# bioinformatics-ua/polus

Hardware: AMD Instinct MI355X
Metric: train samples/sec BioBERT-base NER seq256 (higher is better)
Workload: dtype bf16; 1 GPU; BERT-base (L=12,H=768,A=12,I=3072,V=28996) token classification C=4, seq_len=256, 64 samples/GPU, AdamW lr 5e-5 wd 0.01 warm-up 10%, dropout 0.1 (hidden + attention) (BASELINE.json configs[2] per-GPU shape), random-init weights; global_batch=64, seq_len=256, parallelism=dp1, grad_allreduce=none

## Files before the change

### polus_amd/csrc/attention.hip

```cpp
#include "common.h"

namespace {

constexpr int D = 64;
constexpr int BLK = 64;
constexpr float MASK_NEG = -10000.0f;
constexpr float LOG2E = 1.4426950408889634f, LN2 = 0.6931471805599453f;

template <typename T> struct TileCfg;
template <> struct TileCfg<bf16_t> { static constexpr int RS = 160, EPC = 8, LOG_CPR = 3, NLOAD = 2; };
template <> struct TileCfg<float> { static constexpr int RS = 288, EPC = 4, LOG_CPR = 4, NLOAD = 4; };

template <typename T, int NT = 256>
__device__ __forceinline__ void tile_load(unsigned char* tile, const T* __restrict__ base, long ld, int row0,
                                          int nrows, int col0, int tid) {
    constexpr int LOG = TileCfg<T>::LOG_CPR;
#pragma unroll
    for (int k = 0; k < TileCfg<T>::NLOAD; ++k) {
        int c = tid + NT * k;
        int r = c >> LOG, ch = c & ((1 << LOG) - 1);
        uint4 v = make_uint4(0, 0, 0, 0);
        if (row0 + r < nrows)
            v = *reinterpret_cast<const uint4*>(base + (long)(row0 + r) * ld + col0 + ch * TileCfg<T>::EPC);
        *reinterpret_cast<uint4*>(tile + r * TileCfg<T>::RS + ch * 16) = v;
// ... 37 lines not shown

__device__ __forceinline__ void frag_from_acc(Frag<bf16_t>& f, const f32x4& t0, const f32x4& t1) {
    f.v[0] = (bf16_t)t0[0]; f.v[1] = (bf16_t)t0[1]; f.v[2] = (bf16_t)t0[2]; f.v[3] = (bf16_t)t0[3];
    f.v[4] = (bf16_t)t1[0]; f.v[5] = (bf16_t)t1[1]; f.v[6] = (bf16_t)t1[2]; f.v[7] = (bf16_t)t1[3];
}
__device__ __forceinline__ void frag_from_acc(Frag<float>& f, const f32x4& t0, const f32x4& t1) {
    f.v[0] = t0[0]; f.v[1] = t0[1]; f.v[2] = t0[2]; f.v[3] = t0[3];
    f.v[4] = t1[0]; f.v[5] = t1[1]; f.v[6] = t1[2]; f.v[7] = t1[3];
}

__device__ __forceinline__ float col_max(float v) { v = fmaxf(v, __shfl_xor(v, 16, 64)); return fmaxf(v, __shfl_xor(v, 32, 64)); }
__device__ __forceinline__ float col_sum(float v) { v += __shfl_xor(v, 16, 64); return v + __shfl_xor(v, 32, 64); }

template <typename T>
__device__ __forceinline__ void store_acc_T(T* __restrict__ out, long ld, int row, int col0, const f32x4 (&o)[4],
                                            float mul, int g, bool valid) {
    if (!valid) return;
#pragma unroll
    for (int dt = 0; dt < 4; ++dt) {
        float v[4] = {o[dt][0] * mul, o[dt][1] * mul, o[dt][2] * mul, o[dt][3] * mul};
        store4<T>(out + (long)row * ld + col0 + dt * 16 + 4 * g, v);
    }
}

struct AttnArgs {
    const void* qkv; const int32_t* mask; void* ctx; float* lse;
    const void* dctx; const float* delta; void* dqkv;
    int B, S, A, H;
    float scale;
    unsigned drop_thresh, drop_seed;
    float drop_inv;
    const PolusDyn* dyn;
    int debug;
};

__device__ __forceinline__ float key_bias(const int32_t* mask, int b, int S, int key) {
    if (key >= S) return -INFINITY;
    if (!mask) return 0.0f;
    return (1.0f - (float)mask[(long)b * S + key]) * MASK_NEG;
}

template <typename T, int NW>
__global__ __launch_bounds__(64 * NW) void attn_fwd_kernel(AttnArgs p) {
    if (p.drop_thresh) p.drop_seed = polus_eff_seed(p.drop_seed, p.dyn);
    constexpr int QB = 16 * NW, NT = 64 * NW;
    extern __shared__ __attribute__((aligned(16))) unsigned char smem[];
    unsigned char* Kc = smem;
    unsigned char* Vc = smem + QB * TileCfg<T>::RS;
    float* kbc = reinterpret_cast<float*>(smem + 2 * QB * TileCfg<T>::RS);
    const int tid = threadIdx.x, lane = tid & 63, wid = tid >> 6, i = lane & 15, g = lane >> 4;
    const int q0 = blockIdx.x * QB, h = blockIdx.y, b = blockIdx.z;
    const int S = p.S, H = p.H;
    const long ld = 3L * H;
    const T* qkv = static_cast<const T*>(p.qkv) + (long)b * S * ld;
    const int q = q0 + wid * 16 + i;
    const bool qvalid = q < S;

    Frag<T> qf[2];
#pragma unroll
    for (int sub = 0; sub < 2; ++sub)
        frag_global<T>(qf[sub], qkv + (long)q * ld + h * D + sub * 32 + 8 * g, qvalid);

    const float scale2 = p.scale * LOG2E;
    float m = -1e30f, l = 0.f;
    f32x4 o[4];
#pragma unroll
    for (int dt = 0; dt < 4; ++dt) o[dt] = (f32x4){0.f, 0.f, 0.f, 0.f};
// ... 117 lines not shown

    auto issue_block = [&](int j) {
        unsigned char* st = ring + (j & 3) * FWD_STAGE;
#pragma unroll
        for (int e = 0; e < PPW; ++e) {
            const int piece = wid + e * NW;
            const int row = min(j * BLK + (piece & 7) * 8 + r8, S - 1);
            dma16(qkv + (long)row * ld + (piece < 8 ? H : 2 * H) + h * D + src_chunk, st + piece * 1024);
        }
    };
    const int nblk = (S + BLK - 1) / BLK;
    if (p.mask)
        for (int k0 = wid * 64; k0 < S; k0 += 64 * NW)
            dma4(p.mask + (long)b * S + min(k0 + lane, S - 1), reinterpret_cast<unsigned char*>(kbc) + k0 * 4);
    {
        unsigned char* qs = ring + 3 * FWD_STAGE;
#pragma unroll
        for (int e = 0; e < 2; ++e) {
            const int piece = wid + e * NW;
            dma16(qkv + (long)min(q0 + piece * 8 + r8, S - 1) * ld + h * D + src_chunk, qs + piece * 1024);
        }
    }
#pragma unroll
    for (int j = 0; j < 3; ++j) if (j < nblk) issue_block(j);
    wait_blocks_left<PPW>(min(nblk, 3));
    __builtin_amdgcn_s_barrier();
    Frag<T> qf[2];
    {
        const int row = wid * 16 + i;
#pragma unroll
        for (int sub = 0; sub < 2; ++sub)
            qf[sub].v = *reinterpret_cast<const bf16x8*>(ring + 3 * FWD_STAGE + row * 128 + (((sub * 4 + g) ^ (row & 7)) * 16));
    }
    for (int t = tid; t < nblk * BLK; t += NT) {
        float bias = 0.0f;
        if (p.mask) bias = (1.0f - (float)reinterpret_cast<const int*>(kbc)[t]) * MASK_NEG;
        kbc[t] = t < S ? bias * LOG2E : -INFINITY;
    }
    wait_lgkm();
    __builtin_amdgcn_s_barrier();
    if (nblk > 3) issue_block(3);
    int issued = min(nblk, 4);

    const float scale2 = p.scale * LOG2E;
    float m = -1e30f, l = 0.f;
    f32x4 o[4];
#pragma unroll
    for (int dt = 0; dt < 4; ++dt) o[dt] = (f32x4){0.f, 0.f, 0.f, 0.f};
    const int kx = i & 7;
    const int k_off0 = i * 128 + ((g ^ kx) * 16), k_off1 = i * 128 + (((4 + g) ^ kx) * 16);
    const int vrow = 4 * g + (i >> 2), vx = vrow & 7;
    const int v_base = vrow * 128 + (i & 1) * 8, v_c = (i & 3) >> 1;

    for (int j0 = 0; j0 < nblk; j0 += 2) {
        const bool two = j0 + 1 < nblk;
        f32x4 s[2][4];
#pragma unroll
        for (int jj = 0; jj < 2; ++jj) {
            if (jj == 0 || two) {
                wait_blocks_left<PPW>(issued - 1 - (j0 + jj));
                __builtin_amdgcn_s_barrier();
                const unsigned char* Kt = ring + ((j0 + jj) & 3) * FWD_STAGE;
#pragma unroll
                for (int kt = 0; kt < 4; ++kt) {
                    s[jj][kt] = (f32x4){0.f, 0.f, 0.f, 0.f};
                    Frag<T> a0, a1;
                    a0.v = *reinterpret_cast<const bf16x8*>(Kt + kt * 2048 + k_off0);
                    a1.v = *reinterpret_cast<const bf16x8*>(Kt + kt * 2048 + k_off1);
                    mma16(s[jj][kt], a0, qf[0]);
                    mma16(s[jj][kt], a1, qf[1]);
                }
            } else {
#pragma unroll
                for (int kt = 0; kt < 4; ++kt) s[jj][kt] = (f32x4){-INFINITY, -INFINITY, -INFINITY, -INFINITY};
            }
        }
        float mx = -INFINITY;
#pragma unroll
        for (int jj = 0; jj < 2; ++jj)
            if (jj == 0 || two) {
#pragma unroll
                for (int kt = 0; kt < 4; ++kt) {
                    const f32x4 kb = *reinterpret_cast<const f32x4*>(kbc + (j0 + jj) * BLK + kt * 16 + 4 * g);
#pragma unroll
                    for (int r = 0; r < 4; ++r) s[jj][kt][r] = fmaf(s[jj][kt][r], scale2, kb[r]);
                    mx = fmaxf(mx, fmaxf(fmaxf(s[jj][kt][0], s[jj][kt][1]), fmaxf(s[jj][kt][2], s[jj][kt][3])));
                }
            }
        mx = col_max2(mx);
        const float m_new = fmaxf(m, mx);
        const float alpha = __builtin_amdgcn_exp2f(m - m_new);
        m = m_new;
        float rs = 0.f;
        Frag<T> pf[2][2];
#pragma unroll
        for (int jj = 0; jj < 2; ++jj) {
#pragma unroll
            for (int kt = 0; kt < 4; ++kt)
#pragma unroll
                for (int r = 0; r < 4; ++r) { s[jj][kt][r] = __builtin_amdgcn_exp2f(s[jj][kt][r] - m_new); rs += s[jj][kt][r]; }
            if (p.drop_thresh) {
                const unsigned rowb = (((unsigned)b * p.A + h) * S + (unsigned)q) * S + (j0 + jj) * BLK + 4 * g;
#pragma unroll
                for (int kt = 0; kt < 4; ++kt) {
                    float t4[4] = {s[jj][kt][0], s[jj][kt][1], s[jj][kt][2], s[jj][kt][3]};
                    polus_dropout_run<4>(t4, p.drop_seed, rowb + kt * 16, p.drop_thresh, p.drop_inv, (S & 3) == 0);
                    s[jj][kt] = (f32x4){t4[0], t4[1], t4[2], t4[3]};
                }
            }
            frag_from_acc(pf[jj][0], s[jj][0], s[jj][1]);
            frag_from_acc(pf[jj][1], s[jj][2], s[jj][3]);
        }
        l = l * alpha + rs;
#pragma unroll
        for (int dt = 0; dt < 4; ++dt)
#pragma unroll
            for (int r = 0; r < 4; ++r) o[dt][r] *= alpha;
#pragma unroll
        for (int jj = 0; jj < 2; ++jj) {
            if (jj == 0 || two) {
                const unsigned char* Vt = ring + ((j0 + jj) & 3) * FWD_STAGE + BLK * 128 + v_base;
#pragma unroll
                for (int ks = 0; ks < 2; ++ks)
#pragma unroll
                    for (int dt = 0; dt < 4; ++dt) {
                        const unsigned char* vp = Vt + ks * 4096 + (((2 * dt + v_c) ^ vx) * 16);
                        const s16x4 lo = lds_tr16(vp), hi = lds_tr16(vp + 16 * 128);
                        typedef short s16x8 __attribute__((ext_vector_type(8)));
                        const s16x8 w = {lo[0], lo[1], lo[2], lo[3], hi[0], hi[1], hi[2], hi[3]};
                        Frag<T> va;
                        va.v = __builtin_bit_cast(bf16x8, w);
                        mma16(o[dt], va, pf[jj][ks]);
                    }
            }
        }
        if (j0 + 4 < nblk) {
            wait_lgkm();
            __builtin_amdgcn_s_barrier();
            issue_block(j0 + 4);
            ++issued;
            if (j0 + 5 < nblk) { issue_block(j0 + 5); ++issued; }
        }
    }
    l = col_sum2(l);
    const float inv_l = 1.0f / l;
    wait_lgkm();
    __builtin_amdgcn_s_barrier();
    unsigned char* ot = ring + wid * 2048;
#pragma unroll
    for (int dt = 0; dt < 4; ++dt) {
        float v[4] = {o[dt][0] * inv_l, o[dt][1] * inv_l, o[dt][2] * inv_l, o[dt][3] * inv_l};
        store4<T>(reinterpret_cast<T*>(ot + i * 128 + (((2 * dt + (g >> 1)) ^ (i & 7)) * 16) + (g & 1) * 8), v);
    }
    wait_lgkm();
    T* ctx = static_cast<T*>(p.ctx) + (long)b * S * H;
#pragma unroll
    for (int t = 0; t < 2; ++t) {
        const int row = 8 * t + r8, qq = q0 + wid * 16 + row;
        const uint4 v = *reinterpret_cast<const uint4*>(ot + row * 128 + (lane & 7) * 16);
        if (qq < S) *reinterpret_cast<uint4*>(ctx + (long)qq * H + h * D + (((lane & 7) ^ (row & 7)) * 8)) = v;
    }
    if (q < S && g == 0) p.lse[((long)b * p.A + h) * S + q] = m * LN2 + __logf(l);
}

template <typename T, int NW>
__global__ __launch_bounds__(64 * NW) void attn_bwd_dq_kernel(AttnArgs p) {
    if (p.drop_thresh) p.drop_seed = polus_eff_seed(p.drop_seed, p.dyn);
    constexpr int QB = 16 * NW, NT = 64 * NW;
    extern __shared__ __attribute__((aligned(16))) unsigned char smem[];
    unsigned char* Kc = smem;
    unsigned char* Vc = smem + QB * TileCfg<T>::RS;
    float* kbc = reinterpret_cast<float*>(smem + 2 * QB * TileCfg<T>::RS);
    const int tid = threadIdx.x, lane = tid & 63, wid = tid >> 6, i = lane & 15, g = lane >> 4;
    const int q0 = blockIdx.x * QB, h = blockIdx.y, b = blockIdx.z;
    const int S = p.S, H = p.H;
    const long ld = 3L * H;
    const T* qkv = static_cast<const T*>(p.qkv) + (long)b * S * ld;
    const T* dctx = static_cast<const T*>(p.dctx) + (long)b * S * H;
// ... 192 lines not shown
template <int NW>
__global__ __launch_bounds__(64 * NW) void attn_bwd_fused_kernel(AttnArgs p) {
    typedef bf16_t T;
    constexpr int S = 16 * NW, NT = 64 * NW, RS = TileCfg<T>::RS, NKB = S / KBLK, TPW = 16 / NW;
    if (p.drop_thresh) p.drop_seed = polus_eff_seed(p.drop_seed, p.dyn);
    extern __shared__ __attribute__((aligned(16))) unsigned char smem[];
    unsigned char* Qc = smem;
    unsigned char* Oc = Qc + S * RS;
    unsigned char* Kc = Oc + S * RS;
    unsigned char* Vc = Kc + 2 * KBLK * RS;
    unsigned char* Ps = Vc + 2 * KBLK * RS;
    unsigned char* Ds = Ps + S * RSS;
    float* kbc = reinterpret_cast<float*>(Ds + S * RSS);
    const int tid = threadIdx.x, lane = tid & 63, wid = tid >> 6, i = lane & 15, g = lane >> 4;
    const int h = blockIdx.x, b = blockIdx.y;
    const int H = p.H;
    const long ld = 3L * H;
    const T* qkv = static_cast<const T*>(p.qkv) + (long)b * S * ld;
    const T* dctx = static_cast<const T*>(p.dctx) + (long)b * S * H;
    T* dqkv = static_cast<T*>(p.dqkv) + (long)b * S * ld;
    const int q = wid * 16 + i;

    auto load_kv = [&](int kb, int buf) {
        for (int c = tid; c < 2 * KBLK * 8; c += NT) {
            const int which = c >> 8, cc = c & 255, r = cc >> 3, ch = cc & 7;
            const uint4 v = *reinterpret_cast<const uint4*>(qkv + (long)(kb * KBLK + r) * ld + (1 + which) * H + h * D + ch * 8);
            *reinterpret_cast<uint4*>((which ? Vc : Kc) + (buf * KBLK + r) * RS + ch * 16) = v;
        }
    };
    tile_load<T, NT>(Qc, qkv, ld, 0, S, h * D, tid);
    tile_load<T, NT>(Oc, dctx, H, 0, S, h * D, tid);
    load_kv(0, 0);
    if (tid < S) kbc[tid] = key_bias(p.mask, b, S, tid) * LOG2E;

    Frag<T> qf[2], dof[2];
#pragma unroll
    for (int sub = 0; sub < 2; ++sub) {
        frag_global<T>(qf[sub], qkv + (long)q * ld + h * D + sub * 32 + 8 * g, true);
        frag_global<T>(dof[sub], dctx + (long)q * H + h * D + sub * 32 + 8 * g, true);
    }
    const long stat = ((long)b * p.A + h) * S + q;
    const float lse2 = p.lse[stat] * LOG2E;
    const float scale2 = p.scale * LOG2E;
    float dl = 0.f;
    {
        const T* ctx = static_cast<const T*>(p.ctx) + (long)b * S * H;
#pragma unroll
        for (int sub = 0; sub < 2; ++sub) {
            Frag<T> of;
            frag_global<T>(of, ctx + (long)q * H + h * D + sub * 32 + 8 * g, true);
#pragma unroll
            for (int j = 0; j < 8; ++j) dl += (float)of.v[j] * (float)dof[sub].v[j];
        }
        dl = col_sum(dl);
    }
    f32x4 dq[4];
#pragma unroll
    for (int dt = 0; dt < 4; ++dt) dq[dt] = (f32x4){0.f, 0.f, 0.f, 0.f};
    __syncthreads();

    for (int kb = 0; kb < NKB; ++kb) {
        const int cur = kb & 1;
        const unsigned char* Kt = Kc + cur * KBLK * RS;
        const unsigned char* Vt = Vc + cur * KBLK * RS;
        if (kb + 1 < NKB) load_kv(kb + 1, cur ^ 1);
        f32x4 s[2], dp[2];
#pragma unroll
        for (int kt = 0; kt < 2; ++kt) {
            s[kt] = (f32x4){0.f, 0.f, 0.f, 0.f};
            dp[kt] = (f32x4){0.f, 0.f, 0.f, 0.f};
#pragma unroll
            for (int sub = 0; sub < 2; ++sub) {
                Frag<T> a;
                frag_row<T>(a, Kt, kt * 16 + i, sub, g);
                mma16(s[kt], a, qf[sub]);
                frag_row<T>(a, Vt, kt * 16 + i, sub, g);
                mma16(dp[kt], a, dof[sub]);
            }
        }
        const unsigned rowb = (((unsigned)b * p.A + h) * S + (unsigned)q) * S + kb * KBLK + 4 * g;
#pragma unroll
        for (int kt = 0; kt < 2; ++kt) {
            float pd[4], dsv[4];
            bool keep[4] = {true, true, true, true};
            if (p.drop_thresh) {
                polus_keep4(p.drop_seed, rowb + kt * 16, p.drop_thresh, keep);
            }
#pragma unroll
            for (int r = 0; r < 4; ++r) {
                const float pr = __builtin_amdgcn_exp2f(fmaf(s[kt][r], scale2, kbc[kb * KBLK + kt * 16 + 4 * g + r]) - lse2);
                const float pk = keep[r] ? pr * p.drop_inv : 0.f;
                const float dpe = keep[r] ? dp[kt][r] * p.drop_inv : 0.f;
                pd[r] = pk;
                dsv[r] = pr * (dpe - dl) * p.scale;
                s[kt][r] = dsv[r];
            }
            const int st_off = kt * (S * 32) + q * 32 + ((g ^ ((q >> 2) & 3)) * 8);
            store4<T>(reinterpret_cast<T*>(Ps + st_off), pd);
// ... 5 lines not shown
#pragma unroll
            for (int dt = 0; dt < 4; ++dt) {
                Frag<T> ka;
                frag_tr(ka, Kt, 0, dt * 16, i, g);
                mma16(dq[dt], ka, dsb);
            }
        }
        __syncthreads();
#pragma unroll
        for (int e = 0; e < TPW; ++e) {
            const int t = wid * TPW + e;
            const int type = t >> 3, dt = (t >> 1) & 3, ktile = t & 1;
            const unsigned char* At = type ? Oc : Qc;
            const unsigned char* Bt = type ? Ps : Ds;
            f32x4 acc = (f32x4){0.f, 0.f, 0.f, 0.f};
#pragma unroll
            for (int qs = 0; qs < S / 32; ++qs) {
                Frag<T> a, bb;
                frag_tr(a, At, qs * 32, dt * 16, i, g);
                {
                    const unsigned char* bp = Bt + ktile * (S * 32) + (qs * 32 + 4 * g + (i >> 2)) * 32 + (((i & 3) ^ g) * 8);
                    const s16x4 lo = lds_tr16(bp), hi = lds_tr16(bp + 16 * 32);
                    typedef short s16x8 __attribute__((ext_vector_type(8)));
                    const s16x8 w = {lo[0], lo[1], lo[2], lo[3], hi[0], hi[1], hi[2], hi[3]};
                    bb.v = __builtin_bit_cast(bf16x8, w);
                }
                mma16(acc, a, bb);
            }
            float v[4] = {acc[0], acc[1], acc[2], acc[3]};
            store4<T>(dqkv + (long)(kb * KBLK + ktile * 16 + i) * ld + (type ? 2 * H : H) + h * D + dt * 16 + 4 * g, v);
        }
        __syncthreads();
    }
    store_acc_T<T>(dqkv, ld, q, h * D, dq, 1.0f, g, true);
}

typedef __attribute__((address_space(3))) unsigned char lds_u8;
typedef int v2i_t __attribute__((ext_vector_type(2)));
__device__ __forceinline__ unsigned lds_off(const unsigned char* p) { return (unsigned)(unsigned long)(const lds_u8*)p; }
template <int ROW16>
__device__ __forceinline__ void tr_pair_asm(Frag<bf16_t>& f, unsigned addr) {
    v2i_t lo, hi;
    asm volatile("ds_read_b64_tr_b16 %0, %2\n\tds_read_b64_tr_b16 %1, %2 offset:%3" : "=&v"(lo), "=&v"(hi) : "v"(addr), "n"(ROW16));
    typedef int v4i_t __attribute__((ext_vector_type(4)));
    const v4i_t w = {lo[0], lo[1], hi[0], hi[1]};
    f.v = __builtin_bit_cast(bf16x8, w);
}
__device__ __forceinline__ void ds_read128_asm(Frag<bf16_t>& f, unsigned addr) {
    typedef int v4i_t __attribute__((ext_vector_type(4)));
    v4i_t w;
    asm volatile("ds_read_b128 %0, %1" : "=&v"(w) : "v"(addr));
    f.v = __builtin_bit_cast(bf16x8, w);
}
__device__ __forceinline__ uint2 ds_read64_asm(unsigned addr) {
    v2i_t w;
    asm volatile("ds_read_b64 %0, %1" : "=&v"(w) : "v"(addr));
    return make_uint2((unsigned)w[0], (unsigned)w[1]);
}
__device__ __forceinline__ void lds_fence() {
    asm volatile("s_waitcnt lgkmcnt(0)" ::: "memory");
    __builtin_amdgcn_sched_barrier(0);
}
template <int R> __device__ __forceinline__ unsigned quad_bcast(unsigned v) {
    return (unsigned)__builtin_amdgcn_mov_dpp((int)v, R | (R << 2) | (R << 4) | (R << 6), 0xF, 0xF, true);
}


constexpr int Q64_KB = 64;
template <int NW> struct Q64Cfg {
    static constexpr int S = 16 * NW;
    static constexpr int OFF_O = S * 128, OFF_K = 2 * S * 128, OFF_V = OFF_K + Q64_KB * 128, OFF_P = OFF_V + Q64_KB * 128,
                         OFF_D = OFF_P + 4 * S * 32, OFF_B = OFF_D + 4 * S * 32, SMEM = OFF_B + S * 4;
};

template <int NW>
__global__ __launch_bounds__(64 * NW, 4) void attn_bwd_q64_kernel(AttnArgs p) {
    typedef bf16_t T;
    typedef Q64Cfg<NW> C;
    constexpr int S = C::S, NT = 64 * NW, NKB = S / Q64_KB;
    constexpr int KVP = 16 / NW;
    constexpr int COMBOS = NW >= 8 ? 1 : 8 / NW;
    constexpr int KTW = NW == 16 ? 2 : 4;
    if (p.drop_thresh) p.drop_seed = polus_eff_seed(p.drop_seed, p.dyn);
    extern __shared__ __attribute__((aligned(16))) unsigned char smem[];
    unsigned char* Qi = smem;
    unsigned char* Oi = smem + C::OFF_O;
    unsigned char* Kb = smem + C::OFF_K;
    unsigned char* Vb = smem + C::OFF_V;
    unsigned char* Ps = smem + C::OFF_P;
    unsigned char* Ds = smem + C::OFF_D;
    float* kbc = reinterpret_cast<float*>(smem + C::OFF_B);
    const int tid = threadIdx.x, lane = tid & 63, i = lane & 15, g = lane >> 4;
    const int wid = __builtin_amdgcn_readfirstlane(tid >> 6);
    const int h = blockIdx.x, b = blockIdx.y;
    const int H = p.H;
    const long ld = 3L * H;
    const T* qkv = static_cast<const T*>(p.qkv) + (long)b * S * ld;
    const T* dctx = static_cast<const T*>(p.dctx) + (long)b * S * H;
    T* dqkv = static_cast<T*>(p.dqkv) + (long)b * S * ld;
    const int q = wid * 16 + i;
    const int r8 = lane >> 3, src_chunk = ((lane & 7) ^ r8) * 8;

    auto issue_kv = [&](int kb) {
#pragma unroll
        for (int e = 0; e < KVP; ++e) {
            const int piece = wid + e * NW;
            const long row = (long)(kb * Q64_KB + (piece & 7) * 8 + r8) * ld + h * D + src_chunk;
            dma16(qkv + row + (piece < 8 ? H : 2 * H), (piece < 8 ? Kb : Vb) + (piece & 7) * 1024);
        }
    };
#pragma unroll
    for (int e = 0; e < 2; ++e) {
        const int piece = wid + e * NW;
        dma16(qkv + (long)(piece * 8 + r8) * ld + h * D + src_chunk, Qi + piece * 1024);
        dma16(dctx + (long)(piece * 8 + r8) * H + h * D + src_chunk, Oi + piece * 1024);
    }
    issue_kv(0);
    if (tid < S) kbc[tid] = key_bias(p.mask, b, S, tid) * LOG2E;
    const long stat = ((long)b * p.A + h) * S + q;
    const float lse2 = p.lse[stat] * LOG2E;
    const float scale2 = p.scale * LOG2E;
    Frag<T> of[2];
    {
        const T* ctx = static_cast<const T*>(p.ctx) + (long)b * S * H;
#pragma unroll
        for (int sub = 0; sub < 2; ++sub) frag_global<T>(of[sub], ctx + (long)q * H + h * D + sub * 32 + 8 * g, true);
    }
    wait_vm<0>();
    wait_lgkm();
    __builtin_amdgcn_s_barrier();
    const int qoff0 = q * 128 + ((g ^ (q & 7)) * 16), qoff1 = q * 128 + (((4 + g) ^ (q & 7)) * 16);
    float dl = 0.f;
    {
        Frag<T> dof[2];
        ds_read128_asm(dof[0], lds_off(Oi + qoff0));
        ds_read128_asm(dof[1], lds_off(Oi + qoff1));
        lds_fence();
#pragma unroll
        for (int sub = 0; sub < 2; ++sub)
#pragma unroll
            for (int j = 0; j < 8; ++j) dl += (float)of[sub].v[j] * (float)dof[sub].v[j];
        dl = col_sum(dl);
    }
    f32x4 dq[4];
#pragma unroll
    for (int dt = 0; dt < 4; ++dt) dq[dt] = (f32x4){0.f, 0.f, 0.f, 0.f};

    const int rr0 = i * 128 + ((g ^ (i & 7)) * 16), rr1 = i * 128 + (((4 + g) ^ (i & 7)) * 16);
    const int trow = 4 * g + (i >> 2), tx = trow & 7, thalf = (i & 1) * 8, tc = (i & 3) >> 1;
    const int st_w = q * 32 + ((g ^ ((q >> 2) & 3)) * 8);
    const int st_r = trow * 32 + (((i & 3) ^ g) * 8);

    for (int kb = 0; kb < NKB; ++kb) {
        f32x4 s[4];
        Frag<T> qf[2], dof[2];
        ds_read128_asm(qf[0], lds_off(Qi + qoff0));
        ds_read128_asm(qf[1], lds_off(Qi + qoff1));
        ds_read128_asm(dof[0], lds_off(Oi + qoff0));
        ds_read128_asm(dof[1], lds_off(Oi + qoff1));
        const unsigned rowb = (((unsigned)b * p.A + h) * S + (unsigned)q) * S + kb * Q64_KB + 4 * g;
#pragma unroll
        for (int kt = 0; kt < 4; ++kt) {
            Frag<T> ka[2], va[2];
            ds_read128_asm(ka[0], lds_off(Kb + kt * 2048 + rr0));
            ds_read128_asm(ka[1], lds_off(Kb + kt * 2048 + rr1));
            ds_read128_asm(va[0], lds_off(Vb + kt * 2048 + rr0));
            ds_read128_asm(va[1], lds_off(Vb + kt * 2048 + rr1));
            lds_fence();
            f32x4 dp = (f32x4){0.f, 0.f, 0.f, 0.f};
            s[kt] = (f32x4){0.f, 0.f, 0.f, 0.f};
            mma16(s[kt], ka[0], qf[0]);
            mma16(s[kt], ka[1], qf[1]);
            mma16(dp, va[0], dof[0]);
            mma16(dp, va[1], dof[1]);
            float pd[4], dsv[4];
            bool keep[4] = {true, true, true, true};
            if (p.drop_thresh) polus_keep4(p.drop_seed, rowb + kt * 16, p.drop_thresh, keep);
            const f32x4 kbv = *reinterpret_cast<const f32x4*>(kbc + kb * Q64_KB + kt * 16 + 4 * g);
#pragma unroll
            for (int r = 0; r < 4; ++r) {
                const float pr = __builtin_amdgcn_exp2f(fmaf(s[kt][r], scale2, kbv[r]) - lse2);
                const float pk = keep[r] ? pr * p.drop_inv : 0.f;
                const float dpe = keep[r] ? dp[r] * p.drop_inv : 0.f;
                pd[r] = pk;
                dsv[r] = pr * (dpe - dl) * p.scale;
                s[kt][r] = dsv[r];
            }
            store4<T>(reinterpret_cast<T*>(Ps + kt * (S * 32) + st_w), pd);
            store4<T>(reinterpret_cast<T*>(Ds + kt * (S * 32) + st_w), dsv);
        }
        {
            Frag<T> kT[2][4];
#pragma unroll
            for (int ks = 0; ks < 2; ++ks)
#pragma unroll
                for (int dt = 0; dt < 4; ++dt)
                    tr_pair_asm<16 * 128>(kT[ks][dt], lds_off(Kb + (ks * 32 + trow) * 128 + (((2 * dt + tc) ^ tx) * 16) + thalf));
            lds_fence();
#pragma unroll
            for (int ks = 0; ks < 2; ++ks) {
                Frag<T> dsb;
                frag_from_acc(dsb, s[2 * ks], s[2 * ks + 1]);
#pragma unroll
                for (int dt = 0; dt < 4; ++dt) mma16(dq[dt], kT[ks][dt], dsb);
            }
        }
        wait_lgkm();
        __builtin_amdgcn_s_barrier();
        if (kb + 1 < NKB) issue_kv(kb + 1);
#pragma unroll
        for (int c = 0; c < COMBOS; ++c) {
            const int combo = NW == 16 ? (wid >> 1) : wid * COMBOS + c;
            const int type = combo >> 2, dt = combo & 3, kt0 = NW == 16 ? (wid & 1) * 2 : 0;
            const unsigned char* At = type ? Oi : Qi;
            const unsigned char* Bt = type ? Ps : Ds;
            constexpr int QH = (S / 32) < 4 ? (S / 32) : 4;
            f32x4 acc[KTW];
#pragma unroll
            for (int k2 = 0; k2 < KTW; ++k2) acc[k2] = (f32x4){0.f, 0.f, 0.f, 0.f};
#pragma unroll
            for (int q0 = 0; q0 < S / 32; q0 += QH) {
                Frag<T> af[QH];
#pragma unroll
                for (int qs = 0; qs < QH; ++qs)
                    tr_pair_asm<16 * 128>(af[qs], lds_off(At + ((q0 + qs) * 32 + trow) * 128 + (((2 * dt + tc) ^ tx) * 16) + thalf));
#pragma unroll
                for (int k2 = 0; k2 < KTW; ++k2) {
                    Frag<T> bf[QH];
#pragma unroll
                    for (int qs = 0; qs < QH; ++qs)
                        tr_pair_asm<16 * 32>(bf[qs], lds_off(Bt + (kt0 + k2) * (S * 32) + (q0 + qs) * 32 * 32 + st_r));
                    lds_fence();
#pragma unroll
                    for (int qs = 0; qs < QH; ++qs) mma16(acc[k2], af[qs], bf[qs]);
                }
            }
#pragma unroll
            for (int k2 = 0; k2 < KTW; ++k2) {
                float v[4] = {acc[k2][0], acc[k2][1], acc[k2][2], acc[k2][3]};
                store4<T>(dqkv + (long)(kb * Q64_KB + (kt0 + k2) * 16 + i) * ld + (type ? 2 * H : H) + h * D + dt * 16 + 4 * g, v);
            }
        }
        if (kb + 1 < NKB) wait_vm<COMBOS * KTW>();
        wait_lgkm();
        __builtin_amdgcn_s_barrier();
    }
    store_acc_T<T>(dqkv, ld, q, h * D, dq, 1.0f, g, true);
}

constexpr int KR_KEYS = 256, KR_QS = 32, KR_RING = 4;
constexpr int KR_KV = KR_KEYS * 128;
constexpr int KR_SLICE = KR_QS * 128;
constexpr int KR_DS = 2 * KR_KEYS * 32;
constexpr int KR_OFF_RING = 2 * KR_KV, KR_OFF_DS = KR_OFF_RING + KR_RING * 2 * KR_SLICE, KR_OFF_DQ = KR_OFF_DS + 2 * KR_DS,
              KR_OFF_STAT = KR_OFF_DQ + 2 * KR_SLICE;

__global__ __launch_bounds__(512, 2) void attn_bwd_kres_kernel(AttnArgs p, float* __restrict__ dq_slabs) {
    typedef bf16_t T;
    constexpr int NT = 512;
    if (p.drop_thresh) p.drop_seed = polus_eff_seed(p.drop_seed, p.dyn);
    extern __shared__ __attribute__((aligned(16))) unsigned char smem[];
    unsigned char* Kimg = smem;
    unsigned char* Vimg = smem + KR_KV;
    unsigned char* ring = smem + KR_OFF_RING;
    unsigned char* dsb = smem + KR_OFF_DS;
    unsigned char* dqb = smem + KR_OFF_DQ;
    float* lsec = reinterpret_cast<float*>(smem + KR_OFF_STAT);
    const int S = p.S, H = p.H;
    float* deltac = lsec + S;
    const int tid = threadIdx.x, lane = tid & 63, i = lane & 15, g = lane >> 4;
    const int wid = __builtin_amdgcn_readfirstlane(tid >> 6);
    const int kb = blockIdx.x, h = blockIdx.y, b = blockIdx.z;
    const int key0 = kb * KR_KEYS;
    const long ld = 3L * H;
    const T* qkv = static_cast<const T*>(p.qkv) + (long)b * S * ld;
    const T* dctx = static_cast<const T*>(p.dctx) + (long)b * S * H;
    T* dqkv = static_cast<T*>(p.dqkv) + (long)b * S * ld;
    const int r8 = lane >> 3, src_chunk = ((lane & 7) ^ r8) * 8;
    const int nsl = S / KR_QS;
// ... 250 lines not shown
    return POLUS_OK;
}

}

namespace {
enum AttnFwdRoute { FWD_DMA_4 = 1, FWD_DMA_8, FWD_WIDE_BF16_8, FWD_WIDE_F32_4 };
enum AttnBwdRoute { BWD_FUSED_4 = 1, BWD_FUSED_8, BWD_Q64_16, BWD_KRES_ONE, BWD_KRES_SLABS, BWD_TWO_BF16, BWD_TWO_F32 };

AttnFwdRoute attn_fwd_route(int dtype, int S) {
    if (dtype != POLUS_BF16) return FWD_WIDE_F32_4;
    if (S > FWD_MAX_S) return FWD_WIDE_BF16_8;
    return S >= 96 ? FWD_DMA_8 : FWD_DMA_4;
}

int attn_kres_blocks(int S) { return S % KR_KEYS == 0 && S <= 2048 ? S / KR_KEYS : 0; }

AttnBwdRoute attn_bwd_route(int dtype, int S) {
    if (dtype != POLUS_BF16) return BWD_TWO_F32;
    if (!polus_cfg().attn_fused) return BWD_TWO_BF16;
    const int kres = polus_cfg().attn_bwd_kres, nkb = attn_kres_blocks(S);
    if (kres && nkb > 1) return BWD_KRES_SLABS;
    if (kres >= 2 && nkb == 1) return BWD_KRES_ONE;
    if (S == 256) return BWD_Q64_16;
    if (S == 128) return BWD_FUSED_8;
    if (S == 64) return BWD_FUSED_4;
    return BWD_TWO_BF16;
}

int attn_args(const char* who, AttnArgs& a, int B, int S, int n_heads, float drop_p, uint32_t seed) {
    POLUS_REQUIRE(drop_p >= 0.f && drop_p < 1.f && (long)B * n_heads * S * S < (1LL << 32), "%s: bad dropout arguments", who);
    a.B = B; a.S = S; a.A = n_heads; a.H = n_heads * D; a.scale = 0.125f;
    a.drop_thresh = drop_p > 0.f ? polus_drop_thresh(drop_p) : 0u; a.drop_seed = seed; a.drop_inv = 1.0f / (1.0f - drop_p); a.dyn = polus_dyn();
    return POLUS_OK;
}

template <auto Kern, typename T, int NW>
int launch_wide(const char* who, const AttnArgs& a, hipStream_t st) {
    constexpr int QB = 16 * NW;
    const size_t lds = 2 * (size_t)QB * TileCfg<T>::RS + QB * 4;
    return polus_launch_lds<Kern>(who, dim3((a.S + QB - 1) / QB, a.A, a.B), dim3(64 * NW), lds, lds, st, a);
}
template <int NW>
int launch_fwd_dma(const AttnArgs& a, hipStream_t st) {
    const size_t lds_max = FWD_RING * FWD_STAGE + (FWD_MAX_S + 64 * NW) * 4;
    const size_t lds = FWD_RING * FWD_STAGE + (size_t)((a.S + 64 * NW - 1) / (64 * NW)) * 64 * NW * 4;
    return polus_launch_lds<attn_fwd_dma_kernel<NW>>("polus_attention_fwd", dim3((a.S + 16 * NW - 1) / (16 * NW), a.A, a.B), dim3(64 * NW), lds_max, lds, st, a);
}
template <int NW>
int launch_q64(const AttnArgs& a, hipStream_t st) {
    return polus_launch_lds<attn_bwd_q64_kernel<NW>>("polus_attention_bwd(one pass, 64-key blocks)", dim3(a.A, a.B), dim3(64 * NW), Q64Cfg<NW>::SMEM, Q64Cfg<NW>::SMEM, st, a);
}
template <int NW>
int launch_fused(const AttnArgs& a, hipStream_t st) {
    const size_t lds = 2 * (size_t)a.S * TileCfg<bf16_t>::RS + 4 * (size_t)KBLK * TileCfg<bf16_t>::RS + 2 * (size_t)a.S * RSS + (size_t)a.S * 4;
    return polus_launch_lds<attn_bwd_fused_kernel<NW>>("polus_attention_bwd(fused)", dim3(a.A, a.B), dim3(64 * NW), lds, lds, st, a);
}
int launch_kres(const AttnArgs& a, float* slabs, hipStream_t st) {
    const int nkb = a.S / KR_KEYS;
    const size_t lds = KR_OFF_STAT + 2 * (size_t)a.S * sizeof(float);
    int rc = polus_launch_lds<attn_bwd_kres_kernel>("polus_attention_bwd(key-resident)", dim3(nkb, a.A, a.B), dim3(512), 160 * 1024, lds, st, a, slabs);
    if (rc != POLUS_OK || !slabs) return rc;
    hipLaunchKernelGGL(attn_bwd_dq_finish_kernel, dim3(1024), dim3(256), 0, st, slabs, static_cast<bf16_t*>(a.dqkv), (long)a.B * a.S, a.H, nkb);
    POLUS_CHECK_LAUNCH("polus_attention_bwd(dQ slabs)");
    return POLUS_OK;
}
template <typename T, int NW>
int launch_two_kernel(const AttnArgs& a, hipStream_t st) {
    int rc = launch_wide<attn_bwd_dq_kernel<T, NW>, T, NW>("polus_attention_bwd(dq)", a, st);
    if (rc != POLUS_OK) return rc;
    hipLaunchKernelGGL(attn_bwd_dkv_kernel<T>, dim3((a.S + BLK - 1) / BLK, a.A, a.B), dim3(256), 0, st, a);
    POLUS_CHECK_LAUNCH("polus_attention_bwd(dkv)");
    return POLUS_OK;
}
}

extern "C" int polus_attention_route(int dtype, int S, int* fwd, int* bwd) {
    POLUS_REQUIRE(dtype == POLUS_F32 || dtype == POLUS_BF16, "polus_attention_route: bad dtype %d", dtype);
    POLUS_REQUIRE(S >= 1 && fwd && bwd, "polus_attention_route: bad arguments (S=%d)", S);
    *fwd = attn_fwd_route(dtype, S);
    *bwd = attn_bwd_route(dtype, S);
    return POLUS_OK;
}

extern "C" int polus_attention_fwd(int dtype, const void* qkv, const int32_t* mask, void* ctx, float* lse,
                                   int B, int S, int n_heads, int head_dim, float drop_p, uint32_t seed, void* stream) {
    int rc = check_common("polus_attention_fwd", dtype, B, S, n_heads, head_dim);
    if (rc) return rc;
// ... 51 lines not shown
```

### polus_amd/csrc/common.h

```cpp
#pragma once
#include <hip/hip_runtime.h>
#include <stdint.h>
#include <stdio.h>
#include <string.h>
#include <math.h>

#include "../../include/polus_hip.h"

typedef __bf16 bf16_t;
typedef __bf16 bf16x8 __attribute__((ext_vector_type(8)));
typedef __bf16 bf16x4 __attribute__((ext_vector_type(4)));
typedef short s16x4 __attribute__((ext_vector_type(4)));
typedef float f32x4 __attribute__((ext_vector_type(4)));

void polus_set_error(const char* fmt, ...);
#define POLUS_FAIL(...) do { polus_set_error(__VA_ARGS__); return POLUS_ERR_INVALID; } while (0)
#define POLUS_REQUIRE(cond, ...) do { if (!(cond)) { polus_set_error(__VA_ARGS__); return POLUS_ERR_INVALID; } } while (0)
#define POLUS_CHECK_LAUNCH(name) do { hipError_t e__ = hipGetLastError(); \
    if (e__ != hipSuccess) { polus_set_error("%s: launch failed: %s", name, hipGetErrorString(e__)); return POLUS_ERR_HIP; } } while (0)
#define POLUS_HIP(call) do { hipError_t e__ = (call); \
    if (e__ != hipSuccess) { polus_set_error("%s failed: %s", #call, hipGetErrorString(e__)); return POLUS_ERR_HIP; } } while (0)

template <auto Kern, typename... A>
int polus_launch_lds(const char* who, dim3 grid, dim3 block, size_t lds_max, size_t lds, hipStream_t st, const A&... args) {
    static bool attr_done = false;
    if (!attr_done) {
        POLUS_HIP(hipFuncSetAttribute(reinterpret_cast<const void*>(Kern), hipFuncAttributeMaxDynamicSharedMemorySize, (int)lds_max));
        attr_done = true;
    }
    hipLaunchKernelGGL(Kern, grid, block, lds, st, args...);
    POLUS_CHECK_LAUNCH(who);
    return POLUS_OK;
}

static inline size_t polus_dtype_size(int dt) { return dt == POLUS_BF16 ? 2 : 4; }
static inline bool polus_aligned16(const void* p) { return (((uintptr_t)p) & 15) == 0; }

struct PolusCfg {
    int gemm_pp;
    int gemm_v1;
    int dw_ungrouped;
    int dw_fused_reduce;
    int ln_bwd_blocks;
    int ln_fin_single;
    int gemm_ring128;
    int gemm_auto_split;
    int ln_halfwave;
    int gemm_order;
    int gemm_persist;
    int reserve_cus;
    int attn_bwd_kres;
    int attn_debug;
    int dw_streamk;
    int dw_sk_cus;
    int dw_sk_delta;
    int attn_fused;
};
const PolusCfg& polus_cfg();
int polus_num_cus();
int polus_reserved_cus();

struct PolusDyn { uint32_t salt; float lr, lr_t; uint32_t pad; };
const PolusDyn* polus_dyn();
__device__ __forceinline__ uint32_t polus_eff_seed(uint32_t seed, const PolusDyn* dyn) {
    if (!dyn) return seed;
    uint32_t x = seed + dyn->salt;
    x ^= x >> 15;
    return x * 0x2C1B3C6Du;
}

template <typename T> __device__ __forceinline__ float to_f(T x);
template <> __device__ __forceinline__ float to_f<float>(float x) { return x; }
template <> __device__ __forceinline__ float to_f<bf16_t>(bf16_t x) { return (float)x; }
template <typename T> __device__ __forceinline__ T from_f(float x);
template <> __device__ __forceinline__ float from_f<float>(float x) { return x; }
template <> __device__ __forceinline__ bf16_t from_f<bf16_t>(float x) { return (bf16_t)x; }

template <typename T> __device__ __forceinline__ void load4(const T* p, float (&v)[4]);
template <> __device__ __forceinline__ void load4<float>(const float* p, float (&v)[4]) {
    float4 t = *reinterpret_cast<const float4*>(p); v[0] = t.x; v[1] = t.y; v[2] = t.z; v[3] = t.w;
}
template <> __device__ __forceinline__ void load4<bf16_t>(const bf16_t* p, float (&v)[4]) {
    bf16x4 t = *reinterpret_cast<const bf16x4*>(p);
    v[0] = (float)t[0]; v[1] = (float)t[1]; v[2] = (float)t[2]; v[3] = (float)t[3];
}
// ... 184 lines not shown
```

### polus_amd/csrc/runtime.hip

```cpp
#include "common.h"
#include <stdarg.h>

static thread_local char g_err[512] = "";

void polus_set_error(const char* fmt, ...) {
    va_list ap;
    va_start(ap, fmt);
    vsnprintf(g_err, sizeof(g_err), fmt, ap);
    va_end(ap);
}

extern "C" const char* polus_last_error(void) { return g_err; }

static PolusCfg g_cfg;
static bool g_cfg_ready = false;
static int env_int(const char* name, int dflt) {
    const char* e = getenv(name);
    return (e && *e) ? atoi(e) : dflt;
}
static void read_cfg() {
    g_cfg.gemm_pp = env_int("POLUS_GEMM_PP", 0);
    g_cfg.gemm_v1 = getenv("POLUS_GEMM_V1") != nullptr;
    g_cfg.dw_ungrouped = getenv("POLUS_DW_UNGROUPED") != nullptr;
    g_cfg.gemm_order = env_int("POLUS_GEMM_ORDER", 4);
    g_cfg.reserve_cus = env_int("POLUS_GEMM_RESERVE_CUS", 0);
    g_cfg.gemm_persist = env_int("POLUS_GEMM_PERSIST", 1);
    g_cfg.dw_fused_reduce = env_int("POLUS_DW_FUSED_REDUCE", 1);
    g_cfg.attn_fused = env_int("POLUS_ATTN_FUSED", 1);
    g_cfg.attn_bwd_kres = env_int("POLUS_ATTN_BWD_KRES", 1);
    g_cfg.attn_debug = env_int("POLUS_ATTN_DEBUG", 0);
    g_cfg.ln_halfwave = env_int("POLUS_LN_HALFWAVE", 1);
    g_cfg.gemm_auto_split = env_int("POLUS_GEMM_AUTO_SPLIT", 1);
    g_cfg.gemm_ring128 = env_int("POLUS_GEMM_RING128", 0);
    g_cfg.ln_bwd_blocks = env_int("POLUS_LN_BWD_BLOCKS", 512);
    g_cfg.ln_fin_single = env_int("POLUS_LN_FIN_SINGLE", 512);
    g_cfg.dw_streamk = env_int("POLUS_DW_STREAMK", 0);
    g_cfg.dw_sk_delta = env_int("POLUS_DW_SK_DELTA", 2);
    g_cfg.dw_sk_cus = env_int("POLUS_DW_SK_CUS", 0);
    g_cfg_ready = true;
}
const PolusCfg& polus_cfg() {
    if (!g_cfg_ready) read_cfg();
    return g_cfg;
}
extern "C" int polus_reload_env(void) { read_cfg(); return POLUS_OK; }

int polus_num_cus() {
    static int n = 0;
    if (!n) {
        int dev = 0; hipDeviceProp_t prop;
        if (hipGetDevice(&dev) == hipSuccess && hipGetDeviceProperties(&prop, dev) == hipSuccess) n = prop.multiProcessorCount;
        if (n <= 0) n = 256;
    }
    return n;
}
static int g_reserve_on = 1;
extern "C" int polus_set_reserve_active(int on) { g_reserve_on = on != 0; return POLUS_OK; }
int polus_reserved_cus() { return g_reserve_on ? polus_cfg().reserve_cus : 0; }

static const PolusDyn* g_dyn = nullptr;
const PolusDyn* polus_dyn() { return g_dyn; }
extern "C" int polus_set_dynamic_params(const void* dev_block16) {
    POLUS_REQUIRE(dev_block16 == nullptr || polus_aligned16(dev_block16), "polus_set_dynamic_params: the block must be 16-byte aligned");
// ... 246 lines not shown
```

Baseline: 5386 samples/s.

## Skip fully-padded key blocks in attention forward and backward kernels

```diff
diff --git a/polus_amd/csrc/attention.hip b/polus_amd/csrc/attention.hip
--- a/polus_amd/csrc/attention.hip
+++ b/polus_amd/csrc/attention.hip
@@ -93,7 +93,32 @@
     float drop_inv;
     const PolusDyn* dyn;
     int debug;
+    int kskip;
 };
+
+__device__ __forceinline__ int kext_of_ballot(unsigned long long live, int base) {
+    return live ? base + 64 - __builtin_clzll(live) : 0;
+}
+template <int NWORDS>
+__device__ __forceinline__ int kext_fold(const int* words, bool masked, int S) {
+    typedef int kx4_t __attribute__((ext_vector_type(4)));
+    const unsigned addr = (unsigned)(unsigned long)(const __attribute__((address_space(3))) int*)words;
+    int k = 0;
+#pragma unroll
+    for (int w = 0; w < NWORDS; w += 4) {
+        kx4_t v;
+        asm volatile("ds_read_b128 %0, %1 offset:%2\n\ts_waitcnt lgkmcnt(0)" : "=&v"(v) : "v"(addr), "n"(w * 4));
+        k = max(k, max(max(v[0], v[1]), max(v[2], v[3])));
+    }
+    return __builtin_amdgcn_readfirstlane(masked && k > 0 ? k : S);
+}
+template <int NT>
+__device__ __forceinline__ void zero_dkv_rows(bf16_t* __restrict__ dqkv, long ld, int row0, int S, int H, int h, int tid) {
+    for (int c = tid; c < (S - row0) * 16; c += NT) {
+        const int r = row0 + (c >> 4), which = (c >> 3) & 1, ch = c & 7;
+        *reinterpret_cast<uint4*>(dqkv + (long)r * ld + (1 + which) * H + h * D + ch * 8) = make_uint4(0, 0, 0, 0);
+    }
+}
 
 __device__ __forceinline__ float key_bias(const int32_t* mask, int b, int S, int key) {
     if (key >= S) return -INFINITY;
@@ -277,15 +302,23 @@
         for (int sub = 0; sub < 2; ++sub)
             qf[sub].v = *reinterpret_cast<const bf16x8*>(ring + 3 * FWD_STAGE + row * 128 + (((sub * 4 + g) ^ (row & 7)) * 16));
     }
+    int* kext = reinterpret_cast<int*>(kbc) + (S + NT - 1) / NT * NT;
+    int kw = 0;
     for (int t = tid; t < nblk * BLK; t += NT) {
         float bias = 0.0f;
-        if (p.mask) bias = (1.0f - (float)reinterpret_cast<const int*>(kbc)[t]) * MASK_NEG;
+        int mk = 0;
+        if (p.mask) { mk = reinterpret_cast<const int*>(kbc)[t]; bias = (1.0f - (float)mk) * MASK_NEG; }
         kbc[t] = t < S ? bias * LOG2E : -INFINITY;
-    }
+        const unsigned long long live = __ballot(t < S && mk != 0);
+        if (live) kw = kext_of_ballot(live, t - lane);
+    }
+    if (lane == 0) kext[wid] = kw;
     wait_lgkm();
     __builtin_amdgcn_s_barrier();
-    if (nblk > 3) issue_block(3);
-    int issued = min(nblk, 4);
+    const int kend = kext_fold<NW>(kext, p.mask != nullptr, S);
+    const int nblk_eff = p.kskip ? (kend + BLK - 1) / BLK : nblk;
+    if (nblk_eff > 3) issue_block(3);
+    int issued = min(nblk, 3) + (nblk_eff > 3);
 
     const float scale2 = p.scale * LOG2E;
     float m = -1e30f, l = 0.f;
@@ -297,8 +330,8 @@
     const int vrow = 4 * g + (i >> 2), vx = vrow & 7;
     const int v_base = vrow * 128 + (i & 1) * 8, v_c = (i & 3) >> 1;
 
-    for (int j0 = 0; j0 < nblk; j0 += 2) {
-        const bool two = j0 + 1 < nblk;
+    for (int j0 = 0; j0 < nblk_eff; j0 += 2) {
+        const bool two = j0 + 1 < nblk_eff;
         f32x4 s[2][4];
 #pragma unroll
         for (int jj = 0; jj < 2; ++jj) {
@@ -315,9 +348,6 @@
                     mma16(s[jj][kt], a0, qf[0]);
                     mma16(s[jj][kt], a1, qf[1]);
                 }
-            } else {
-#pragma unroll
-                for (int kt = 0; kt < 4; ++kt) s[jj][kt] = (f32x4){-INFINITY, -INFINITY, -INFINITY, -INFINITY};
             }
         }
         float mx = -INFINITY;
@@ -340,6 +370,7 @@
         Frag<T> pf[2][2];
 #pragma unroll
         for (int jj = 0; jj < 2; ++jj) {
+            if (jj == 1 && !two) continue;
 #pragma unroll
             for (int kt = 0; kt < 4; ++kt)
 #pragma unroll
@@ -379,16 +410,17 @@
                     }
             }
         }
-        if (j0 + 4 < nblk) {
+        if (j0 + 4 < nblk_eff) {
             wait_lgkm();
             __builtin_amdgcn_s_barrier();
             issue_block(j0 + 4);
             ++issued;
-            if (j0 + 5 < nblk) { issue_block(j0 + 5); ++issued; }
+            if (j0 + 5 < nblk_eff) { issue_block(j0 + 5); ++issued; }
         }
     }
     l = col_sum2(l);
     const float inv_l = 1.0f / l;
+    wait_vm<0>();
     wait_lgkm();
     __builtin_amdgcn_s_barrier();
     unsigned char* ot = ring + wid * 2048;
@@ -647,6 +679,11 @@
     tile_load<T, NT>(Oc, dctx, H, 0, S, h * D, tid);
     load_kv(0, 0);
     if (tid < S) kbc[tid] = key_bias(p.mask, b, S, tid) * LOG2E;
+    int* kext = reinterpret_cast<int*>(kbc + S);
+    if (wid < 4) {
+        const unsigned long long live = __ballot(tid < S && p.mask && p.mask[(long)b * S + tid] != 0);
+        if (lane == 0) kext[wid] = kext_of_ballot(live, wid * 64);
+    }
 
     Frag<T> qf[2], dof[2];
 #pragma unroll
@@ -673,12 +710,14 @@
 #pragma unroll
     for (int dt = 0; dt < 4; ++dt) dq[dt] = (f32x4){0.f, 0.f, 0.f, 0.f};
     __syncthreads();
-
-    for (int kb = 0; kb < NKB; ++kb) {
+    const int kend = kext_fold<4>(kext, p.mask != nullptr, S);
+    const int nkb_eff = p.kskip ? (kend + KBLK - 1) / KBLK : NKB;
+
+    for (int kb = 0; kb < nkb_eff; ++kb) {
         const int cur = kb & 1;
         const unsigned char* Kt = Kc + cur * KBLK * RS;
         const unsigned char* Vt = Vc + cur * KBLK * RS;
-        if (kb + 1 < NKB) load_kv(kb + 1, cur ^ 1);
+        if (kb + 1 < nkb_eff) load_kv(kb + 1, cur ^ 1);
         f32x4 s[2], dp[2];
 #pragma unroll
         for (int kt = 0; kt < 2; ++kt) {
@@ -750,6 +789,7 @@
         }
         __syncthreads();
     }
+    zero_dkv_rows<NT>(dqkv, ld, nkb_eff * KBLK, S, H, h, tid);
     store_acc_T<T>(dqkv, ld, q, h * D, dq, 1.0f, g, true);
 }
 
@@ -788,7 +828,7 @@
 template <int NW> struct Q64Cfg {
     static constexpr int S = 16 * NW;
     static constexpr int OFF_O = S * 128, OFF_K = 2 * S * 128, OFF_V = OFF_K + Q64_KB * 128, OFF_P = OFF_V + Q64_KB * 128,
-                         OFF_D = OFF_P + 4 * S * 32, OFF_B = OFF_D + 4 * S * 32, SMEM = OFF_B + S * 4;
+                         OFF_D = OFF_P + 4 * S * 32, OFF_B = OFF_D + 4 * S * 32, OFF_X = OFF_B + S * 4, SMEM = OFF_X + 16;
 };
 
 template <int NW>
@@ -808,6 +848,7 @@
     unsigned char* Ps = smem + C::OFF_P;
     unsigned char* Ds = smem + C::OFF_D;
     float* kbc = reinterpret_cast<float*>(smem + C::OFF_B);
+    int* kext = reinterpret_cast<int*>(smem + C::OFF_X);
     const int tid = threadIdx.x, lane = tid & 63, i = lane & 15, g = lane >> 4;
     const int wid = __builtin_amdgcn_readfirstlane(tid >> 6);
     const int h = blockIdx.x, b = blockIdx.y;
@@ -835,6 +876,10 @@
     }
     issue_kv(0);
     if (tid < S) kbc[tid] = key_bias(p.mask, b, S, tid) * LOG2E;
+    if (wid < 4) {
+        const unsigned long long live = __ballot(tid < S && p.mask && p.mask[(long)b * S + tid] != 0);
+        if (lane == 0) kext[wid] = kext_of_ballot(live, wid * 64);
+    }
     const long stat = ((long)b * p.A + h) * S + q;
     const float lse2 = p.lse[stat] * LOG2E;
     const float scale2 = p.scale * LOG2E;
@@ -868,8 +913,10 @@
     const int trow = 4 * g + (i >> 2), tx = trow & 7, thalf = (i & 1) * 8, tc = (i & 3) >> 1;
     const int st_w = q * 32 + ((g ^ ((q >> 2) & 3)) * 8);
     const int st_r = trow * 32 + (((i & 3) ^ g) * 8);
-
-    for (int kb = 0; kb < NKB; ++kb) {
+    const int kend = kext_fold<4>(kext, p.mask != nullptr, S);
+    const int nkb_eff = p.kskip ? (kend + Q64_KB - 1) / Q64_KB : NKB;
+
+    for (int kb = 0; kb < nkb_eff; ++kb) {
         f32x4 s[4];
         Frag<T> qf[2], dof[2];
         ds_read128_asm(qf[0], lds_off(Qi + qoff0));
@@ -925,7 +972,7 @@
         }
         wait_lgkm();
         __builtin_amdgcn_s_barrier();
-        if (kb + 1 < NKB) issue_kv(kb + 1);
+        if (kb + 1 < nkb_eff) issue_kv(kb + 1);
 #pragma unroll
         for (int c = 0; c < COMBOS; ++c) {
             const int combo = NW == 16 ? (wid >> 1) : wid * COMBOS + c;
@@ -959,10 +1006,11 @@
                 store4<T>(dqkv + (long)(kb * Q64_KB + (kt0 + k2) * 16 + i) * ld + (type ? 2 * H : H) + h * D + dt * 16 + 4 * g, v);
             }
         }
-        if (kb + 1 < NKB) wait_vm<COMBOS * KTW>();
+        if (kb + 1 < nkb_eff) wait_vm<COMBOS * KTW>();
         wait_lgkm();
         __builtin_amdgcn_s_barrier();
     }
+    zero_dkv_rows<NT>(dqkv, ld, nkb_eff * Q64_KB, S, H, h, tid);
     store_acc_T<T>(dqkv, ld, q, h * D, dq, 1.0f, g, true);
 }
 
@@ -1279,6 +1327,7 @@
     POLUS_REQUIRE(drop_p >= 0.f && drop_p < 1.f && (long)B * n_heads * S * S < (1LL << 32), "%s: bad dropout arguments", who);
     a.B = B; a.S = S; a.A = n_heads; a.H = n_heads * D; a.scale = 0.125f;
     a.drop_thresh = drop_p > 0.f ? polus_drop_thresh(drop_p) : 0u; a.drop_seed = seed; a.drop_inv = 1.0f / (1.0f - drop_p); a.dyn = polus_dyn();
+    a.kskip = polus_cfg().attn_kskip != 0;
     return POLUS_OK;
 }
 
@@ -1290,8 +1339,8 @@
 }
 template <int NW>
 int launch_fwd_dma(const AttnArgs& a, hipStream_t st) {
-    const size_t lds_max = FWD_RING * FWD_STAGE + (FWD_MAX_S + 64 * NW) * 4;
-    const size_t lds = FWD_RING * FWD_STAGE + (size_t)((a.S + 64 * NW - 1) / (64 * NW)) * 64 * NW * 4;
+    const size_t lds_max = FWD_RING * FWD_STAGE + (FWD_MAX_S + 64 * NW) * 4 + NW * 4;
+    const size_t lds = FWD_RING * FWD_STAGE + (size_t)((a.S + 64 * NW - 1) / (64 * NW)) * 64 * NW * 4 + NW * 4;
     return polus_launch_lds<attn_fwd_dma_kernel<NW>>("polus_attention_fwd", dim3((a.S + 16 * NW - 1) / (16 * NW), a.A, a.B), dim3(64 * NW), lds_max, lds, st, a);
 }
 template <int NW>
@@ -1300,7 +1349,7 @@
 }
 template <int NW>
 int launch_fused(const AttnArgs& a, hipStream_t st) {
-    const size_t lds = 2 * (size_t)a.S * TileCfg<bf16_t>::RS + 4 * (size_t)KBLK * TileCfg<bf16_t>::RS + 2 * (size_t)a.S * RSS + (size_t)a.S * 4;
+    const size_t lds = 2 * (size_t)a.S * TileCfg<bf16_t>::RS + 4 * (size_t)KBLK * TileCfg<bf16_t>::RS + 2 * (size_t)a.S * RSS + (size_t)a.S * 4 + 16;
     return polus_launch_lds<attn_bwd_fused_kernel<NW>>("polus_attention_bwd(fused)", dim3(a.A, a.B), dim3(64 * NW), lds, lds, st, a);
 }
 int launch_kres(const AttnArgs& a, float* slabs, hipStream_t st) {
diff --git a/polus_amd/csrc/common.h b/polus_amd/csrc/common.h
--- a/polus_amd/csrc/common.h
+++ b/polus_amd/csrc/common.h
@@ -51,6 +51,7 @@
     int reserve_cus;
     int attn_bwd_kres;
     int attn_debug;
+    int attn_kskip;
     int dw_streamk;
     int dw_sk_cus;
     int dw_sk_delta;
diff --git a/polus_amd/csrc/runtime.hip b/polus_amd/csrc/runtime.hip
--- a/polus_amd/csrc/runtime.hip
+++ b/polus_amd/csrc/runtime.hip
@@ -29,6 +29,7 @@
     g_cfg.attn_fused = env_int("POLUS_ATTN_FUSED", 1);
     g_cfg.attn_bwd_kres = env_int("POLUS_ATTN_BWD_KRES", 1);
     g_cfg.attn_debug = env_int("POLUS_ATTN_DEBUG", 0);
+    g_cfg.attn_kskip = env_int("POLUS_ATTN_KSKIP", 1);
     g_cfg.ln_halfwave = env_int("POLUS_LN_HALFWAVE", 1);
     g_cfg.gemm_auto_split = env_int("POLUS_GEMM_AUTO_SPLIT", 1);
     g_cfg.gemm_ring128 = env_int("POLUS_GEMM_RING128", 0);
```

Result: faster. 5448 samples/s (median of 6 runs) (+1.1%).
